# Electron-Labs/eth-lc-plonky2

Measured on AMD Instinct MI355X. Metric: lc_proofs_per_hour, higher is better.
Workload: dtype u64

## Files before the change

### eth-lc-plonky2_amd/csrc/internal.hpp

```cpp
#pragma once
#include <hip/hip_runtime.h>
#include <functional>
#include <map>
#include <string>
#include <vector>
#include "../../include/lcp2.h"
#include "gl64.hpp"
#include "ntt.hpp"

namespace lcp2 {

struct ProfFamily {
  std::vector<std::pair<hipEvent_t, hipEvent_t>> pending;
  double ms = 0;
  uint64_t launches = 0;
  double bytes = 0;
};

}

struct lcp2_ctx {
  int device = -1;
  hipStream_t stream = nullptr;
  bool own_stream = false;
  std::string last_error;
  lcp2::u64 *d_rc = nullptr;
  std::map<std::string, lcp2::u64 *> tables;
  bool prof_on = false;
  lcp2::ProfFamily fam[LCP2_K_COUNT];
  std::vector<hipEvent_t> event_pool;
  void *pin = nullptr;
  static constexpr size_t PIN_BYTES = 4u << 20;
  hipStream_t copy_stream = nullptr;
  void *scratch[4] = {nullptr, nullptr, nullptr, nullptr};
  size_t scratch_bytes[4] = {0, 0, 0, 0};

  int fail(int code, const std::string &msg) {
    last_error = msg;
    return code;
  }
};

namespace lcp2 {

#define LCP2_HIP(ctx, expr)                                                                  \
  do {                                                                                       \
    hipError_t e_ = (expr);                                                                  \
    if (e_ != hipSuccess)                                                                    \
      return (ctx)->fail(e_ == hipErrorOutOfMemory ? LCP2_E_OOM : LCP2_E_HIP,                \
                         std::string(#expr) + ": " + hipGetErrorString(e_));                 \
  } while (0)
#define LCP2_TRY(expr) do { int rc_ = (expr); if (rc_ != LCP2_OK) return rc_; } while (0)

struct DevBuf {
  void *p = nullptr;
  size_t bytes = 0;
  DevBuf() = default;
  DevBuf(const DevBuf &) = delete;
  DevBuf &operator=(const DevBuf &) = delete;
  DevBuf(DevBuf &&o) noexcept : p(o.p), bytes(o.bytes) { o.p = nullptr; o.bytes = 0; }
  DevBuf &operator=(DevBuf &&o) noexcept {
    if (this != &o) { release(); p = o.p; bytes = o.bytes; o.p = nullptr; o.bytes = 0; }
    return *this;
  }
  ~DevBuf() { release(); }
  hipError_t alloc(size_t n) {
    release();
    if (n == 0) n = 8;
    hipError_t e = hipMalloc(&p, n);
    if (e == hipSuccess) bytes = n; else p = nullptr;
    return e;
  }
  hipError_t ensure(size_t n) { return (p && bytes >= n) ? hipSuccess : alloc(n); }
  void release() { if (p) { (void)hipFree(p); p = nullptr; bytes = 0; } }
  u64 *u() const { return (u64 *)p; }
};

struct ProfScope {
  lcp2_ctx *ctx;
  int family;
  hipEvent_t a = nullptr, b = nullptr;
  ProfScope(lcp2_ctx *c, int fam, double algorithmic_bytes);
  ~ProfScope();
};

int scratch_ensure(lcp2_ctx *ctx, int slot, size_t bytes, void **out);

void launch_poseidon_permute_batch(hipStream_t s, const u64 *in, u64 *out, size_t count, const u64 *rc);
// ... 68 lines not shown
```

### eth-lc-plonky2_amd/csrc/lcp2_core.hip

```cpp
#include <cstring>
#include "internal.hpp"
#include "ntt_host.hpp"
#include "poseidon.hpp"
#include "prover_kernels.hpp"

using namespace lcp2;

extern "C" const char *lcp2_status_str(int s) {
  switch (s) {
    case LCP2_OK: return "ok";
    case LCP2_E_INVALID: return "invalid argument";
    case LCP2_E_NODEVICE: return "no usable HIP device";
    case LCP2_E_HIP: return "HIP runtime error";
    case LCP2_E_OOM: return "out of device memory";
    case LCP2_E_UNSAT: return "witness does not satisfy the circuit";
    case LCP2_E_UNSUPPORTED: return "unsupported";
    case LCP2_E_VERIFY: return "proof rejected";
    default: return "unknown status";
  }
}
extern "C" int lcp2_abi_version(void) { return LCP2_ABI_VERSION; }
extern "C" int lcp2_device_count(void) {
  int n = 0;
  if (hipGetDeviceCount(&n) != hipSuccess) return 0;
// ... 14 lines not shown
    if (d < arity_bits) return LCP2_E_INVALID;
    if (n == LCP2_MAX_FRI_LAYERS) return LCP2_E_UNSUPPORTED;
    p->fri_arity_bits[n++] = arity_bits;
    d -= arity_bits;
  }
  p->num_fri_layers = n;
  return LCP2_OK;
}
extern "C" int lcp2_params_standard(uint32_t degree_bits, uint32_t num_constants, lcp2_params *p) {
  return lcp2_params_config(degree_bits, num_constants, 3, 4, 16, 28, 4, 5, p);
}

extern "C" int lcp2_ctx_create(int device, void *stream, lcp2_ctx **out) { return lcp2_ctx_create_ex(device, stream, 0, out); }
extern "C" int lcp2_ctx_create_ex(int device, void *stream, uint32_t flags, lcp2_ctx **out) {
  if (!out) return LCP2_E_INVALID;
  *out = nullptr;
  if ((flags & ~LCP2_CTX_ORDER_WITH_DEFAULT_STREAM) || ((flags & LCP2_CTX_ORDER_WITH_DEFAULT_STREAM) && stream)) return LCP2_E_INVALID;
  int ndev = 0;
  if (hipGetDeviceCount(&ndev) != hipSuccess || ndev <= 0) return LCP2_E_NODEVICE;
  if (device < 0 || device >= ndev) return LCP2_E_INVALID;
  if (hipSetDevice(device) != hipSuccess) return LCP2_E_NODEVICE;
  lcp2_ctx *ctx = new lcp2_ctx();
  ctx->device = device;
  if (stream) {
    ctx->stream = (hipStream_t)stream;
  } else {
    const unsigned how = (flags & LCP2_CTX_ORDER_WITH_DEFAULT_STREAM) ? hipStreamDefault : hipStreamNonBlocking;
    if (hipStreamCreateWithFlags(&ctx->stream, how) != hipSuccess) { delete ctx; return LCP2_E_HIP; }
    ctx->own_stream = true;
  }
  if (hipHostMalloc(&ctx->pin, lcp2_ctx::PIN_BYTES, hipHostMallocDefault) != hipSuccess) ctx->pin = nullptr;
  u64 rc[POS_RC_WORDS];
  pos_derive_round_constants(rc);
  pos_extend_round_constants(rc);
  if (hipMalloc((void **)&ctx->d_rc, sizeof rc) != hipSuccess ||
      hipMemcpy(ctx->d_rc, rc, sizeof rc, hipMemcpyHostToDevice) != hipSuccess) {
    lcp2_ctx_destroy(ctx);
    return LCP2_E_HIP;
  }
  *out = ctx;
  return LCP2_OK;
}

extern "C" void *lcp2_ctx_stream(lcp2_ctx *ctx) { return ctx ? (void *)ctx->stream : nullptr; }

extern "C" void lcp2_ctx_destroy(lcp2_ctx *ctx) {
  if (!ctx) return;
  (void)hipSetDevice(ctx->device);
  (void)hipStreamSynchronize(ctx->stream);
  for (auto &kv : ctx->tables) (void)hipFree(kv.second);
  for (auto &f : ctx->fam)
    for (auto &pr : f.pending) { (void)hipEventDestroy(pr.first); (void)hipEventDestroy(pr.second); }
  for (auto e : ctx->event_pool) (void)hipEventDestroy(e);
  if (ctx->d_rc) (void)hipFree(ctx->d_rc);
  if (ctx->pin) (void)hipHostFree(ctx->pin);
  for (void *q : ctx->scratch) if (q) (void)hipFree(q);
  if (ctx->copy_stream) { (void)hipStreamSynchronize(ctx->copy_stream); (void)hipStreamDestroy(ctx->copy_stream); }
  if (ctx->own_stream) (void)hipStreamDestroy(ctx->stream);
  delete ctx;
}

extern "C" int lcp2_ctx_sync(lcp2_ctx *ctx) {
  if (!ctx) return LCP2_E_INVALID;
  LCP2_HIP(ctx, hipStreamSynchronize(ctx->stream));
  return LCP2_OK;
}
extern "C" const char *lcp2_last_error(lcp2_ctx *ctx) { return ctx ? ctx->last_error.c_str() : "null context"; }

namespace lcp2 {
static hipEvent_t take_event(lcp2_ctx *ctx) {
  if (!ctx->event_pool.empty()) { hipEvent_t e = ctx->event_pool.back(); ctx->event_pool.pop_back(); return e; }
  hipEvent_t e = nullptr;
  (void)hipEventCreate(&e);
  return e;
}
ProfScope::ProfScope(lcp2_ctx *c, int fam, double algorithmic_bytes) : ctx(c), family(fam) {
  if (!ctx->prof_on) return;
  a = take_event(ctx); b = take_event(ctx);
  ctx->fam[family].bytes += algorithmic_bytes;
  (void)hipEventRecord(a, ctx->stream);
}
ProfScope::~ProfScope() {
  if (!a) return;
  (void)hipEventRecord(b, ctx->stream);
  ctx->fam[family].pending.emplace_back(a, b);
}
static void prof_collect(lcp2_ctx *ctx) {
  (void)hipStreamSynchronize(ctx->stream);
  for (auto &f : ctx->fam) {
    for (auto &pr : f.pending) {
      float ms = 0;
      if (hipEventElapsedTime(&ms, pr.first, pr.second) == hipSuccess) { f.ms += ms; f.launches++; }
      ctx->event_pool.push_back(pr.first); ctx->event_pool.push_back(pr.second);
    }
    f.pending.clear();
  }
}
}

extern "C" int lcp2_prof_enable(lcp2_ctx *ctx, int on) {
  if (!ctx) return LCP2_E_INVALID;
  if (!on) prof_collect(ctx);
  ctx->prof_on = on != 0;
  return LCP2_OK;
}
extern "C" int lcp2_prof_reset(lcp2_ctx *ctx) {
// ... 434 lines not shown
```

### eth-lc-plonky2_amd/csrc/witness_rows.hip

```cpp
#include <cstring>
#include "internal.hpp"
#include "row_stage.hpp"
#include "sha_layout.hpp"
#include "sha_rows.hpp"
#include "pos_rows.hpp"
#include "prover_kernels.hpp"
#include "u32_rows.hpp"
#include "rec_rows.hpp"
#include "pos_plan.hpp"
#include "u32_plan.hpp"

using namespace lcp2;

namespace lcp2 {
int scratch_ensure(lcp2_ctx *ctx, int slot, size_t bytes, void **out) {
  if (ctx->scratch_bytes[slot] < bytes) {
    if (ctx->scratch[slot]) { LCP2_HIP(ctx, hipStreamSynchronize(ctx->stream)); LCP2_HIP(ctx, hipFree(ctx->scratch[slot])); ctx->scratch[slot] = nullptr; ctx->scratch_bytes[slot] = 0; }
    const size_t want = bytes + bytes / 4 + 4096;
    LCP2_HIP(ctx, hipMalloc(&ctx->scratch[slot], want));
    ctx->scratch_bytes[slot] = want;
  }
  *out = ctx->scratch[slot];
  return LCP2_OK;
}
}

namespace {
constexpr size_t ENDS_OK = ~(size_t)0;
size_t ends_problem(const uint32_t *ends, size_t count, size_t total) {
  if (!total) return ENDS_OK;
  for (size_t l = 0; l < count; l++)
    if (ends[l] < (l ? ends[l - 1] : 0) || ends[l] > total) return l;
  return count && ends[count - 1] == total ? ENDS_OK : count;
}
}

static_assert(sizeof(lcp2_sha_job) == sizeof(ShaJobDev) && sizeof(lcp2_cell) == sizeof(CellDev), "ABI structs must match the kernels'");

extern "C" int lcp2_sha256_witness(lcp2_ctx *ctx, const lcp2_sha_job *jobs, size_t njobs, const uint32_t *level_start, uint32_t nlevels,
                                   const uint32_t *words_in, size_t nwords, uint64_t *wires, uint64_t n, uint32_t *digests) {
  if (!ctx || !wires || (njobs && (!jobs || !level_start || nlevels == 0)) || (nwords && !words_in)) return LCP2_E_INVALID;
  if (njobs == 0) return LCP2_OK;
  if (const ShaProblem refused = sha_jobs_problem((const ShaJobDev *)jobs, njobs, level_start, nlevels, nwords, n); refused.problem)
    return ctx->fail(LCP2_E_INVALID, sha_problem_str(refused.problem));
  LCP2_HIP(ctx, hipSetDevice(ctx->device));
  void *d_jobs, *d_words, *d_rec;
  LCP2_TRY(scratch_ensure(ctx, 0, njobs * sizeof(lcp2_sha_job), &d_jobs));
  LCP2_TRY(scratch_ensure(ctx, 1, std::max<size_t>(nwords, 1) * 4, &d_words));
  LCP2_TRY(scratch_ensure(ctx, 2, njobs * (size_t)SHA_REC_WORDS * 4, &d_rec));
  Stage stage{ctx};
  LCP2_TRY(stage.behind(d_jobs, jobs, njobs * sizeof(lcp2_sha_job)));
  if (nwords) LCP2_TRY(stage.behind(d_words, words_in, nwords * 4));
  {
    ProfScope ps(ctx, LCP2_K_SHA256, 96.0 * njobs + 8.0 * 108 * SHA_ROWS * njobs);
    for (uint32_t l = 0; l < nlevels; l++)
      launch_sha_jobs_level(ctx->stream, (const ShaJobDev *)d_jobs, level_start[l], level_start[l + 1] - level_start[l],
                            (const uint32_t *)d_words, (uint32_t *)d_rec);
    launch_sha_fill_rows(ctx->stream, (const ShaJobDev *)d_jobs, (u32)njobs, (const uint32_t *)d_rec, (u64 *)wires, n);
  }
  LCP2_HIP(ctx, hipGetLastError());
  char *back = digests ? stage.room(njobs * 32) : nullptr;
  if (digests)
    LCP2_HIP(ctx, hipMemcpy2DAsync(back ? (void *)back : (void *)digests, 32, (const uint32_t *)d_rec + SHA_REC_DIGEST,
                                   (size_t)SHA_REC_WORDS * 4, 32, njobs, hipMemcpyDeviceToHost, ctx->stream));
  LCP2_HIP(ctx, hipStreamSynchronize(ctx->stream));
  if (back) memcpy(digests, back, njobs * 32);
  return LCP2_OK;
}

extern "C" int lcp2_scatter_cells(lcp2_ctx *ctx, const lcp2_cell *cells, size_t ncells, uint64_t *wires, uint64_t n) {
  if (!ctx || !wires || (ncells && !cells)) return LCP2_E_INVALID;
  if (!ncells) return LCP2_OK;
  if (scatter_cells_problem((const CellDev *)cells, ncells, n) != ncells) return ctx->fail(LCP2_E_INVALID, "scatter: row out of range");
  LCP2_HIP(ctx, hipSetDevice(ctx->device));
  void *d;
  LCP2_TRY(scratch_ensure(ctx, 3, ncells * sizeof(lcp2_cell), &d));
  LCP2_TRY(Stage{ctx}.behind(d, cells, ncells * sizeof(lcp2_cell)));
  launch_scatter_cells(ctx->stream, (const CellDev *)d, ncells, (u64 *)wires, n);
  LCP2_HIP(ctx, hipGetLastError());
  LCP2_HIP(ctx, hipStreamSynchronize(ctx->stream));
  return LCP2_OK;
}

extern "C" int lcp2_poseidon_gate_rows(lcp2_ctx *ctx, const lcp2_poseidon_row *rows, size_t nrows, uint64_t *wires, uint64_t n) {
  static_assert(sizeof(lcp2_poseidon_row) == sizeof(PoseidonRowDev), "row job layouts must agree");
  if (!ctx || !wires || (nrows && !rows)) return LCP2_E_INVALID;
  if (!nrows) return LCP2_OK;
  for (size_t i = 0; i < nrows; i++)
    if (pos_row_problem(((const PoseidonRowDev *)rows)[i], n)) return ctx->fail(LCP2_E_INVALID, "poseidon rows: row out of range or swap flag not boolean");
  LCP2_HIP(ctx, hipSetDevice(ctx->device));
  void *d;
  LCP2_TRY(scratch_ensure(ctx, 0, nrows * sizeof(lcp2_poseidon_row), &d));
  LCP2_TRY(Stage{ctx}.behind(d, rows, nrows * sizeof(lcp2_poseidon_row)));
  launch_poseidon_gate_rows(ctx->stream, (const PoseidonRowDev *)d, nrows, (u64 *)wires, n, ctx->d_rc);
  LCP2_HIP(ctx, hipGetLastError());
  LCP2_HIP(ctx, hipStreamSynchronize(ctx->stream));
  return LCP2_OK;
}

extern "C" int lcp2_u32_gate_rows(lcp2_ctx *ctx, const lcp2_u32_job *jobs, size_t njobs, lcp2_mem jobs_mem, uint64_t *wires, uint64_t n) {
  static_assert(sizeof(lcp2_u32_job) == 24 && sizeof(lcp2_u32_job) == sizeof(U32JobDev), "job layouts must agree");
  static_assert(LCP2_U32_ARITHMETIC == U32_KIND_ARITHMETIC && LCP2_U32_ADD_MANY == U32_KIND_ADD_MANY && LCP2_U32_SUBTRACTION == U32_KIND_SUBTRACTION &&
                LCP2_U32_RANGE_CHECK == U32_KIND_RANGE_CHECK && LCP2_U32_COMPARISON == U32_KIND_COMPARISON, "kind numbering must agree");
  if (!ctx || !wires || (njobs && !jobs)) return LCP2_E_INVALID;
  if (jobs_mem != LCP2_MEM_HOST && jobs_mem != LCP2_MEM_DEVICE) return ctx->fail(LCP2_E_INVALID, "u32 rows: bad lcp2_mem");
  if (!njobs) return LCP2_OK;
  const U32JobDev *list = (const U32JobDev *)jobs;
  if (jobs_mem == LCP2_MEM_HOST)
    for (size_t i = 0; i < njobs; i++)
      if (u32 problem = u32_job_problem(list[i], n))
        return ctx->fail(LCP2_E_INVALID, "u32 rows: job " + std::to_string(i) + ": " + u32_problem_str(problem));
  LCP2_HIP(ctx, hipSetDevice(ctx->device));
  RefusalFlag flag{ctx};
  LCP2_TRY(flag.begin());
  if (jobs_mem == LCP2_MEM_DEVICE) {
    launch_u32_gate_rows(ctx->stream, list, njobs, (u64 *)wires, n, flag.d);
  } else {
    constexpr size_t PIECE = (size_t)1 << 20;
    void *d;
    LCP2_TRY(scratch_ensure(ctx, 0, std::min(njobs, PIECE) * sizeof(lcp2_u32_job), &d));
    for (size_t at = 0; at < njobs; at += PIECE) {
      const size_t count = std::min(PIECE, njobs - at);
      LCP2_TRY(Stage{ctx}.behind(d, list + at, count * sizeof(lcp2_u32_job), njobs <= PIECE));
      launch_u32_gate_rows(ctx->stream, (const U32JobDev *)d, count, (u64 *)wires, n, flag.d);
    }
  }
  return flag.end("u32 rows", u32_problem_str, "the valid jobs are written");
}

namespace {
struct PlanTexts {
  const char *label, *rec_job, *written;
};

int run_plan_rows(lcp2_ctx *ctx, const lcp2_witness_plan_u32 &q, lcp2_mem lists_mem, uint64_t *wires, uint32_t ncols, uint64_t n, const PlanTexts &text) {
  const lcp2_witness_plan &p = q.base;
  const bool host = lists_mem == LCP2_MEM_HOST;
  const RecJobDev *rec = (const RecJobDev *)p.rec_jobs;
  const U32PlanJobDev *u32_jobs = (const U32PlanJobDev *)q.u32_jobs;
  const PosJobDev *pos = (const PosJobDev *)p.pos_jobs;
  const RecOperandDev *ops = (const RecOperandDev *)p.operands;
  const u32 *chain_ends = p.chain_ends;
  auto refused = [&](u32 family, u64 job, u32 problem, bool on_device) {
    return ctx->fail(LCP2_E_INVALID, std::string(text.label) + ": " + (family == 2 ? "u32 job " : family ? "poseidon job " : text.rec_job) + std::to_string(job) + ": " +
                                         (family == 2 ? u32_plan_problem_str(problem) : family ? pos_plan_problem_str(problem) : rec_problem_str(problem)) +
                                         (on_device ? std::string(" (found on the device: ") + text.written + ")" : std::string()));
  };
  if (host)
// ... 103 lines not shown
```

### eth-lc-plonky2_amd/host/builder.cpp

```cpp
#include <cstdio>
#include <algorithm>
#include <atomic>
#include <chrono>
#include <cstdlib>
#include <map>
#include <thread>
#include "host_internal.hpp"

namespace lc {

const uint32_t SHA_K[64] = {
    0x428a2f98, 0x71374491, 0xb5c0fbcf, 0xe9b5dba5, 0x3956c25b, 0x59f111f1, 0x923f82a4, 0xab1c5ed5, 0xd807aa98, 0x12835b01,
    0x243185be, 0x550c7dc3, 0x72be5d74, 0x80deb1fe, 0x9bdc06a7, 0xc19bf174, 0xe49b69c1, 0xefbe4786, 0x0fc19dc6, 0x240ca1cc,
    0x2de92c6f, 0x4a7484aa, 0x5cb0a9dc, 0x76f988da, 0x983e5152, 0xa831c66d, 0xb00327c8, 0xbf597fc7, 0xc6e00bf3, 0xd5a79147,
    0x06ca6351, 0x14292967, 0x27b70a85, 0x2e1b2138, 0x4d2c6dfc, 0x53380d13, 0x650a7354, 0x766a0abb, 0x81c2c92e, 0x92722c85,
    0xa2bfe8a1, 0xa81a664b, 0xc24b8b70, 0xc76c51a3, 0xd192e819, 0xd6990624, 0xf40e3585, 0x106aa070, 0x19a4c116, 0x1e376c08,
    0x2748774c, 0x34b0bcb5, 0x391c0cb3, 0x4ed8aa4a, 0x5b9cca4f, 0x682e6ff3, 0x748f82ee, 0x78a5636f, 0x84c87814, 0x8cc70208,
    0x90befffa, 0xa4506ceb, 0xbef9a3f7, 0xc67178f2};
const uint32_t SHA_IV[8] = {0x6a09e667, 0xbb67ae85, 0x3c6ef372, 0xa54ff53a, 0x510e527f, 0x9b05688c, 0x1f83d9ab, 0x5be0cd19};

static inline uint32_t rotr(uint32_t x, int r) { return (x >> r) | (x << (32 - r)); }

void PartialWitness::set_target(Target t, F value) { entries_.push_back({t.id, value % GOLDILOCKS_P}); }
void PartialWitness::set_hash256_target(const Hash256Target &t, const uint8_t v[32]) {
// ... 693 lines not shown
          if (backoff < 8) backoff++;
          continue;
        }
        idle.fetch_add(1, std::memory_order_acq_rel);
        while (!stop.load(std::memory_order_acquire) && epoch.load(std::memory_order_acquire) == e0) {
          if (idle.load(std::memory_order_acquire) >= active.load(std::memory_order_acquire)) stop.store(true, std::memory_order_release);
          else std::this_thread::yield();
        }
        idle.fetch_sub(1, std::memory_order_acq_rel);
      }
    } catch (...) {
      failure[k] = std::current_exception();
      stop.store(true, std::memory_order_release);
    }
    active.fetch_sub(1, std::memory_order_acq_rel);
  };
  std::vector<std::thread> threads;
  for (unsigned k = 1; k < K; k++) threads.emplace_back(lane_main, k);
  lane_main(0);
  for (auto &t : threads) t.join();
  for (unsigned k = 0; k < K; k++) if (failure[k]) std::rethrow_exception(failure[k]);
  host_ops.clear();
  for (unsigned k = 0; k < K; k++) {
    host_ops.insert(host_ops.end(), mine[k].begin(), mine[k].end());
    cells.insert(cells.end(), lane_cells[k].begin(), lane_cells[k].end());
    pos_rows.insert(pos_rows.end(), lane_rows[k].begin(), lane_rows[k].end());
  }
  std::sort(host_ops.begin(), host_ops.end());
}

void CircuitData::generate_witness_gpu(const PartialWitness &pw, std::vector<F> &public_inputs) {
  Impl *d = impl_.get();
  if (!d->gpu) throw std::runtime_error("generate_witness_gpu needs attach_gpu()");
  const uint64_t n = 1ull << desc_.params.degree_bits;
  Values V(d);
  for (auto &e : pw.entries()) V.set(e.first, e.second, "PartialWitness");
  std::vector<const Op *> host_ops, sha_ops;
  for (const Op &op : d->ops) (op.kind == Op::SHA ? sha_ops : host_ops).push_back(&op);
  std::vector<lcp2_cell> cells;
  std::vector<lcp2_poseidon_row> pos_rows;
  const bool prof = getenv("LCP2_PROF") != nullptr;
  auto now = [] { return std::chrono::steady_clock::now(); };
  auto ms = [](std::chrono::steady_clock::time_point a, std::chrono::steady_clock::time_point b) { return std::chrono::duration<double, std::milli>(b - a).count(); };
  double t_host = 0;
  if (d->host_lanes.lane_of_op.size() != d->ops.size()) {
    unsigned want = 1;
    if (const char *e = getenv("LCP2_HOST_LANES")) want = (unsigned)atoi(e);
    d->host_lanes = plan_host_lanes(d, std::max(1u, std::min(want, 8u)));
  }
  HostPhaseStats st;
  bool recording = !d->gpu_plan.ready;
  GpuWitnessPlan recorded;
  size_t n_batches = 0;
  const auto t_begin = now();
  while (true) {
    const auto t0 = now();
    run_host_phase(d, d->host_lanes, host_ops, V, cells, pos_rows, st);
    t_host += ms(t0, now());
    if (sha_ops.empty()) break;
    const size_t batch_no = n_batches++;
    if (d->gpu_plan.ready && batch_no < d->gpu_plan.batches.size()) {
      const ShaBatchPlan &B = d->gpu_plan.batches[batch_no];
      bool applies = B.ops_left.size() < sha_ops.size();
      std::vector<uint32_t> words(B.word_vars.size());
      for (size_t k = 0; k < words.size() && applies; k++) {
        if (!V.known(B.word_vars[k])) applies = false;
        else words[k] = as_u32(V.val[B.word_vars[k]], "sha256 message word");
      }
      if (applies) {
        std::vector<uint32_t> digests(B.jobs.size() * 8);
        int rc = lcp2_sha256_witness(d->ctx, B.jobs.data(), B.jobs.size(), B.level_start.data(), (uint32_t)B.level_start.size() - 1, words.data(), words.size(),
                                     (uint64_t *)d->d_wires, n, digests.data());
        if (rc != LCP2_OK) throw std::runtime_error(std::string("lcp2_sha256_witness: ") + lcp2_status_str(rc) + " (" + lcp2_last_error(d->ctx) + ")");
        for (size_t k = 0; k < B.jobs.size(); k++)
          for (int w = 0; w < 8; w++) V.set(B.out[k][w], digests[k * 8 + w], "sha256 digest");
        sha_ops.clear();
        for (uint32_t k : B.ops_left) sha_ops.push_back(&d->ops[k]);
        continue;
      }
      d->gpu_plan = GpuWitnessPlan();
      recording = false;
    }
    std::map<uint32_t, uint32_t> produced;
    std::vector<lcp2_sha_job> jobs;
    std::vector<uint32_t> level, words, word_vars;
    std::vector<const Op *> batch, later;
    for (const Op *op : sha_ops) {
      lcp2_sha_job job{};
      job.first_row = op->first_row;
      uint32_t lvl = 0;
      bool ok = true;
      size_t words_mark = words.size();
      for (int i = 0; i < 16 && ok; i++) {
        uint32_t r = d->find(op->in[i]);
        if (V.known(r)) { job.in_src[i] = (int32_t)words.size(); words.push_back(as_u32(V.val[r], "sha256 message word")); word_vars.push_back(r); }
        else {
          auto it = produced.find(r);
          if (it == produced.end()) ok = false;
          else { job.in_src[i] = ~(int32_t)it->second; lvl = std::max(lvl, level[it->second >> 3] + 1); }
        }
      }
      if (!ok) { words.resize(words_mark); word_vars.resize(words_mark); later.push_back(op); continue; }
      uint32_t slot = (uint32_t)jobs.size();
      for (int w = 0; w < 8; w++) produced[d->find(op->out8[w])] = slot * 8 + w;
      jobs.push_back(job); level.push_back(lvl); batch.push_back(op);
    }
    if (jobs.empty()) throw UnsatisfiedError("a generator is waiting for a target that is never set");
    uint32_t nlev = 0;
    for (uint32_t l : level) nlev = std::max(nlev, l + 1);
    std::vector<uint32_t> order(jobs.size()), newslot(jobs.size()), level_start(nlev + 1, 0);
    for (uint32_t l : level) level_start[l + 1]++;
    for (uint32_t l = 0; l < nlev; l++) level_start[l + 1] += level_start[l];
    {
      std::vector<uint32_t> fill(level_start.begin(), level_start.end() - 1);
      for (uint32_t s = 0; s < jobs.size(); s++) { newslot[s] = fill[level[s]]++; order[newslot[s]] = s; }
    }
    std::vector<lcp2_sha_job> sorted(jobs.size());
    for (uint32_t s = 0; s < jobs.size(); s++) {
      lcp2_sha_job j = jobs[s];
      for (int i = 0; i < 16; i++)
        if (j.in_src[i] < 0) { uint32_t ref = (uint32_t)~j.in_src[i]; j.in_src[i] = ~(int32_t)(newslot[ref >> 3] * 8 + (ref & 7)); }
      sorted[newslot[s]] = j;
    }
    std::vector<uint32_t> digests(jobs.size() * 8);
    int rc = lcp2_sha256_witness(d->ctx, sorted.data(), sorted.size(), level_start.data(), nlev, words.data(), words.size(),
                                 (uint64_t *)d->d_wires, n, digests.data());
    if (rc != LCP2_OK) throw std::runtime_error(std::string("lcp2_sha256_witness: ") + lcp2_status_str(rc) + " (" + lcp2_last_error(d->ctx) + ")");
    for (uint32_t s = 0; s < batch.size(); s++)
      for (int w = 0; w < 8; w++) V.set(batch[s]->out8[w], digests[(size_t)newslot[s] * 8 + w], "sha256 digest");
    if (recording) {
      ShaBatchPlan B;
      B.jobs = sorted; B.word_vars = word_vars; B.level_start = level_start;
      for (const Op *op : later) B.ops_left.push_back((uint32_t)(op - d->ops.data()));
      B.out.resize(jobs.size());
      for (uint32_t s = 0; s < batch.size(); s++)
        for (int w = 0; w < 8; w++) B.out[newslot[s]][w] = d->find(batch[s]->out8[w]);
      recorded.batches.push_back(std::move(B));
    }
    sha_ops.swap(later);
  }
  if (!host_ops.empty()) throw UnsatisfiedError("a generator is waiting for a target that is never set");
  const auto t_rows = now();
  int rc = lcp2_poseidon_gate_rows(d->ctx, pos_rows.data(), pos_rows.size(), (uint64_t *)d->d_wires, n);
  if (rc != LCP2_OK) throw std::runtime_error(std::string("lcp2_poseidon_gate_rows: ") + lcp2_status_str(rc) + " (" + lcp2_last_error(d->ctx) + ")");
  if (!d->gpu_plan.ready) {
    GpuWitnessPlan fresh;
    std::vector<bool> listed(d->fill_copies ? d->parent.size() : 0, false);
    for (const CellBinding &c : d->cells) {
      uint32_t g = d->gate_of_row[c.row];
      if (g == G_SHA_ADD || g == G_SHA_ROUND_A || g == G_SHA_ROUND_E || g == G_SHA_SCHED || g == G_POSEIDON) continue;
      const uint32_t root = d->find(c.var);
      if (d->fill_copies) {
        if (listed[root]) continue;
        listed[root] = true;
      }
      fresh.host_cells.push_back(CellBinding{c.row, c.col, root});
    }
    if (recording) { fresh.batches = std::move(recorded.batches); fresh.ready = true; }
    d->gpu_plan = std::move(fresh);
  }
  std::vector<lcp2_cell> &buf = d->cell_buf;
  if (buf.size() != d->gpu_plan.host_cells.size()) {
    if (d->cell_buf_pinned) { lcp2_host_unregister(d->ctx, buf.data()); d->cell_buf_pinned = false; }
    buf.resize(d->gpu_plan.host_cells.size());
    for (size_t k = 0; k < buf.size(); k++) { buf[k].row = d->gpu_plan.host_cells[k].row; buf[k].col = d->gpu_plan.host_cells[k].col; }
    if (!buf.empty()) d->cell_buf_pinned = lcp2_host_register(d->ctx, buf.data(), buf.size() * sizeof(lcp2_cell)) == LCP2_OK;
  }
  for (size_t k = 0; k < buf.size(); k++) {
    const uint32_t var = d->gpu_plan.host_cells[k].var;
    if (!V.known(var)) throw UnsatisfiedError("target has no value: wire cell");
    buf[k].value = V.val[var];
  }
  const auto t_scatter = now();
  d->cells_sent = buf.size() + cells.size();
  if (d->fill_copies) {
    rc = lcp2_witness_fill_copies(d->gpu, buf.data(), buf.size(), LCP2_MEM_HOST, (uint64_t *)d->d_wires, nullptr);
    if (rc == LCP2_OK) rc = lcp2_witness_fill_copies(d->gpu, cells.data(), cells.size(), LCP2_MEM_HOST, (uint64_t *)d->d_wires, nullptr);
    if (rc != LCP2_OK) throw std::runtime_error(std::string("lcp2_witness_fill_copies: ") + lcp2_status_str(rc) + " (" + lcp2_last_error(d->ctx) + ")");
  } else {
    rc = lcp2_scatter_cells(d->ctx, buf.data(), buf.size(), (uint64_t *)d->d_wires, n);
    if (rc == LCP2_OK) rc = lcp2_scatter_cells(d->ctx, cells.data(), cells.size(), (uint64_t *)d->d_wires, n);
    if (rc != LCP2_OK) throw std::runtime_error(std::string("lcp2_scatter_cells: ") + lcp2_status_str(rc));
  }
  if (prof)
    printf("  witness generation %.2f ms: host generators %.2f ms on %u lane(s) (%zu sweeps, %zu visits of %zu ops, %zu PoseidonGate rows), SHA-256 batches %.2f ms, "
           "PoseidonGate rows on the device + cell list %.2f ms, scatter of %zu cells %.2f ms\n",
           ms(t_begin, now()), t_host, d->host_lanes.lanes, st.sweeps, st.visits, d->ops.size(), pos_rows.size(), ms(t_begin, t_rows) - t_host, ms(t_rows, t_scatter), cells.size() + buf.size(), ms(t_scatter, now()));
  public_inputs.clear();
  for (uint32_t v : d->public_inputs) public_inputs.push_back(V.get(v, "public input"));
}

void CircuitData::set_fill_copies(bool on) {
  if (impl_->fill_copies == on) return;
  impl_->fill_copies = on;
  impl_->gpu_plan = GpuWitnessPlan();
}
size_t CircuitData::cells_sent_last() const { return impl_->cells_sent; }

void CircuitData::read_device_witness(std::vector<uint64_t> &wires) const {
  const size_t words = (size_t)desc_.params.num_wires << desc_.params.degree_bits;
  wires.resize(words);
  if (!impl_->d_wires || lcp2_buffer_read(impl_->ctx, wires.data(), impl_->d_wires, words * 8) != LCP2_OK)
    throw std::runtime_error("read_device_witness failed");
}

ProofWithPublicInputs CircuitData::prove(const PartialWitness &pw) {
  if (!impl_->gpu) throw std::runtime_error("CircuitData::prove needs attach_gpu(): there is no CPU prover in this library");
  ProofWithPublicInputs out;
  generate_witness_gpu(pw, out.public_inputs);
  out.proof.assign(lcp2_proof_words(&desc_.params), 0);
  int rc = lcp2_prove(impl_->gpu, (const uint64_t *)impl_->d_wires, LCP2_MEM_DEVICE, out.public_inputs.data(), out.public_inputs.size(),
                      out.proof.data(), out.proof.size());
  if (rc == LCP2_E_UNSAT) throw UnsatisfiedError(std::string("lcp2_prove: ") + lcp2_last_error(impl_->ctx));
  if (rc != LCP2_OK) throw std::runtime_error(std::string("lcp2_prove: ") + lcp2_status_str(rc) + " (" + lcp2_last_error(impl_->ctx) + ")");
  return out;
}

std::string CircuitData::describe_report(const lcp2_witness_report &r) const {
  if (r.gate_violations == 0 && r.copy_violations == 0) return "the witness satisfies every gate and copy constraint";
  auto cell = [](uint64_t row, uint32_t wire) { return "(" + std::to_string(row) + ", " + std::to_string(wire) + ")"; };
  std::string text;
  if (r.gate_violations) {
    const char *name = r.gate_index < desc_.gates.size() && r.gate_index < G_COUNT ? gate_name(r.gate_index) : "gate ?";
    text = "row " + std::to_string(r.gate_row) + ", gate " + name + ", constraint " + std::to_string(r.gate_constraint) + " (" +
           std::to_string(r.gate_violations) + " gate constraints violated)";
  }
  if (r.copy_violations) {
    if (!text.empty()) text += "; ";
    text += "copy constraint " + cell(r.copy_row, r.copy_wire) + " != " +
            (r.copy_to_wire == 0xFFFFFFFFu ? std::string("(no cell: the sigma value is no cell id)") : cell(r.copy_to_row, r.copy_to_wire)) + " (" +
            std::to_string(r.copy_violations) + " cells)";
  }
  return text;
}

static std::string diagnose_on_device(lcp2_ctx *ctx, lcp2_circuit *gpu, const CircuitData &data, const uint64_t *wires, lcp2_mem mem,
                                      const std::vector<F> &public_inputs) {
  lcp2_witness_report report;
  const int rc = lcp2_check_witness(gpu, wires, mem, public_inputs.data(), public_inputs.size(), &report, nullptr, 0);
// ... 57 lines not shown
```

### include/lcp2.h

```cpp
#ifndef LCP2_H
#define LCP2_H
#include <stddef.h>
#include <stdint.h>

#ifdef __cplusplus
extern "C" {
#endif

#define LCP2_ABI_VERSION 2

typedef enum {
  LCP2_OK = 0,
  LCP2_E_INVALID = -1,
  LCP2_E_NODEVICE = -2,
  LCP2_E_HIP = -3,
  LCP2_E_OOM = -4,
  LCP2_E_UNSAT = -5,
  LCP2_E_UNSUPPORTED = -6,
  LCP2_E_VERIFY = -7
} lcp2_status;

typedef enum { LCP2_MEM_HOST = 0, LCP2_MEM_DEVICE = 1 } lcp2_mem;

#define LCP2_MAX_FRI_LAYERS 8
// ... 19 lines not shown

typedef struct lcp2_ctx lcp2_ctx;
typedef struct lcp2_oracle lcp2_oracle;

const char *lcp2_status_str(int status);
int lcp2_abi_version(void);
int lcp2_device_count(void);

int lcp2_ctx_create(int device, void *stream, lcp2_ctx **out);
#define LCP2_CTX_ORDER_WITH_DEFAULT_STREAM 1u
int lcp2_ctx_create_ex(int device, void *stream, uint32_t flags, lcp2_ctx **out);
void lcp2_ctx_destroy(lcp2_ctx *ctx);
int lcp2_ctx_sync(lcp2_ctx *ctx);
void *lcp2_ctx_stream(lcp2_ctx *ctx);
const char *lcp2_last_error(lcp2_ctx *ctx);


int lcp2_poseidon_permute_batch(lcp2_ctx *ctx, const uint64_t *in, uint64_t *out, size_t count, lcp2_mem mem);

enum {
  LCP2_FIELD_MUL = 0,
  LCP2_FIELD_POW7 = 1,
  LCP2_FIELD_ADD = 2,
  LCP2_FIELD_SUB = 3,
  LCP2_FIELD_CANON = 4,
  LCP2_FIELD_ADD_LAZY = 5,
  LCP2_FIELD_SUB_LAZY = 6,
  LCP2_FIELD_SHL = 16
};
int lcp2_field_op_batch(lcp2_ctx *ctx, const uint64_t *a, const uint64_t *b, uint64_t *out, size_t count, uint32_t op, lcp2_mem mem);

int lcp2_merkle_cap(lcp2_ctx *ctx, const uint64_t *leaves, size_t nleaves, size_t leaf_len,
                    uint32_t cap_height, lcp2_mem mem, uint64_t *cap );

int lcp2_ntt_batch(lcp2_ctx *ctx, uint64_t *data, size_t ncols, uint32_t log_n, int inverse,
                   uint64_t shift, lcp2_mem mem);

int lcp2_lde_batch(lcp2_ctx *ctx, const uint64_t *coeffs, uint64_t *out, size_t ncols, uint32_t log_n,
                   uint32_t rate_bits, lcp2_mem mem);

int lcp2_sha256_tree(lcp2_ctx *ctx, const uint8_t *leaves, uint32_t height, size_t trees,
                     uint8_t *nodes, uint32_t *round_trace, lcp2_mem mem);

typedef struct {
  uint32_t first_row;
  int32_t in_src[16];
} lcp2_sha_job;
typedef struct {
  uint32_t row, col;
  uint64_t value;
} lcp2_cell;
int lcp2_sha256_witness(lcp2_ctx *ctx, const lcp2_sha_job *jobs, size_t njobs, const uint32_t *level_start, uint32_t nlevels,
                        const uint32_t *words_in, size_t nwords, uint64_t *wires, uint64_t n, uint32_t *digests);
int lcp2_scatter_cells(lcp2_ctx *ctx, const lcp2_cell *cells, size_t ncells, uint64_t *wires, uint64_t n);
typedef struct {
  uint32_t row;
  uint32_t swap;
  uint64_t in[12];
} lcp2_poseidon_row;
int lcp2_poseidon_gate_rows(lcp2_ctx *ctx, const lcp2_poseidon_row *rows, size_t nrows, uint64_t *wires, uint64_t n);
enum { LCP2_U32_ARITHMETIC = 0, LCP2_U32_ADD_MANY = 1, LCP2_U32_SUBTRACTION = 2, LCP2_U32_RANGE_CHECK = 3, LCP2_U32_COMPARISON = 4 };
typedef struct {
  uint32_t row;
  uint16_t kind;
  uint16_t op;
  uint32_t in[4];
} lcp2_u32_job;
int lcp2_u32_gate_rows(lcp2_ctx *ctx, const lcp2_u32_job *jobs, size_t njobs, lcp2_mem jobs_mem,
                       uint64_t *wires , uint64_t n);

enum { LCP2_REC_ARITHMETIC = 0, LCP2_REC_BASE_SUM, LCP2_REC_ARITHMETIC_EXT, LCP2_REC_MUL_EXT, LCP2_REC_REDUCING,
       LCP2_REC_REDUCING_EXT, LCP2_REC_POSEIDON_MDS, LCP2_REC_RANDOM_ACCESS, LCP2_REC_EXPONENTIATION,
       LCP2_REC_COSET_INTERPOLATION, LCP2_REC_KINDS };
enum { LCP2_REC_IMM = 0, LCP2_REC_CELL = 1 };
typedef struct {
  uint64_t v;
  uint32_t col;
  uint32_t src;
} lcp2_rec_operand;
typedef struct {
  uint32_t row;
  uint16_t kind;
  uint16_t op;
  uint32_t first_operand, reserved;
} lcp2_rec_job;
int lcp2_rec_gate_rows(lcp2_ctx *ctx, const lcp2_rec_job *jobs, size_t njobs,
                       const lcp2_rec_operand *operands, size_t noperands,
                       const uint32_t *level_ends , size_t nlevels,
                       lcp2_mem lists_mem ,
                       uint64_t *wires , uint32_t ncols, uint64_t n);

enum { LCP2_PLAN_IMM = 0, LCP2_PLAN_CELL = 1, LCP2_PLAN_PREV = 2 };
typedef struct { uint32_t row, first_operand; } lcp2_pos_job;
typedef struct {
  const lcp2_rec_job *rec_jobs;  size_t nrec;    const uint32_t *rec_level_ends;
  const lcp2_pos_job *pos_jobs;  size_t npos;
  const uint32_t *chain_ends;    size_t nchains;
  const uint32_t *pos_level_ends;
  const lcp2_rec_operand *operands; size_t noperands;
  size_t nlevels;
} lcp2_witness_plan;
int lcp2_witness_plan_rows(lcp2_ctx *ctx, const lcp2_witness_plan *plan, lcp2_mem lists_mem,
                           uint64_t *wires , uint32_t ncols, uint64_t n);

typedef struct { uint32_t row; uint16_t kind , op; uint32_t first_operand, reserved; } lcp2_u32_plan_job;
typedef struct {
  lcp2_witness_plan base;
  const lcp2_u32_plan_job *u32_jobs; size_t nu32;
  const uint32_t *u32_level_ends;
} lcp2_witness_plan_u32;
int lcp2_witness_plan_rows_u32(lcp2_ctx *ctx, const lcp2_witness_plan_u32 *plan, lcp2_mem lists_mem,
                               uint64_t *wires , uint32_t ncols, uint64_t n);

// ... 204 lines not shown
```

Before: 9350.

## Overlap host cell-value gathering with SHA-256 witness batches and merge syncs

The SHA-256 witness call is split into begin/end, so the host fills the known wire-cell values into the pinned cell buffer while the device runs the SHA batch. Cells whose values are not yet known are tracked in a late list and retried on later passes. The PoseidonGate rows and the host-cell scatter are now queued together behind one stream synchronize instead of two. This adds per-context pending state and more complex bookkeeping on the host in exchange for less serial host work and fewer syncs.

```diff
diff --git a/eth-lc-plonky2_amd/csrc/internal.hpp b/eth-lc-plonky2_amd/csrc/internal.hpp
--- a/eth-lc-plonky2_amd/csrc/internal.hpp
+++ b/eth-lc-plonky2_amd/csrc/internal.hpp
@@ -34,6 +34,13 @@
   hipStream_t copy_stream = nullptr;
   void *scratch[4] = {nullptr, nullptr, nullptr, nullptr};
   size_t scratch_bytes[4] = {0, 0, 0, 0};
+  hipEvent_t sha_done = nullptr;
+  struct ShaPending {
+    bool open = false;
+    const char *staged = nullptr;
+    uint32_t *digests = nullptr;
+    size_t bytes = 0;
+  } sha_pending;
 
   int fail(int code, const std::string &msg) {
     last_error = msg;
diff --git a/eth-lc-plonky2_amd/csrc/lcp2_core.hip b/eth-lc-plonky2_amd/csrc/lcp2_core.hip
--- a/eth-lc-plonky2_amd/csrc/lcp2_core.hip
+++ b/eth-lc-plonky2_amd/csrc/lcp2_core.hip
@@ -90,6 +90,7 @@
   for (auto &f : ctx->fam)
     for (auto &pr : f.pending) { (void)hipEventDestroy(pr.first); (void)hipEventDestroy(pr.second); }
   for (auto e : ctx->event_pool) (void)hipEventDestroy(e);
+  if (ctx->sha_done) (void)hipEventDestroy(ctx->sha_done);
   if (ctx->d_rc) (void)hipFree(ctx->d_rc);
   if (ctx->pin) (void)hipHostFree(ctx->pin);
   for (void *q : ctx->scratch) if (q) (void)hipFree(q);
diff --git a/eth-lc-plonky2_amd/csrc/witness_rows.hip b/eth-lc-plonky2_amd/csrc/witness_rows.hip
--- a/eth-lc-plonky2_amd/csrc/witness_rows.hip
+++ b/eth-lc-plonky2_amd/csrc/witness_rows.hip
@@ -37,9 +37,10 @@
 
 static_assert(sizeof(lcp2_sha_job) == sizeof(ShaJobDev) && sizeof(lcp2_cell) == sizeof(CellDev), "ABI structs must match the kernels'");
 
-extern "C" int lcp2_sha256_witness(lcp2_ctx *ctx, const lcp2_sha_job *jobs, size_t njobs, const uint32_t *level_start, uint32_t nlevels,
-                                   const uint32_t *words_in, size_t nwords, uint64_t *wires, uint64_t n, uint32_t *digests) {
+extern "C" int lcp2_sha256_witness_begin(lcp2_ctx *ctx, const lcp2_sha_job *jobs, size_t njobs, const uint32_t *level_start, uint32_t nlevels,
+                                         const uint32_t *words_in, size_t nwords, uint64_t *wires, uint64_t n, uint32_t *digests) {
   if (!ctx || !wires || (njobs && (!jobs || !level_start || nlevels == 0)) || (nwords && !words_in)) return LCP2_E_INVALID;
+  if (ctx->sha_pending.open) return ctx->fail(LCP2_E_INVALID, "sha256 witness: the batch begun before has not been ended");
   if (njobs == 0) return LCP2_OK;
   if (const ShaProblem refused = sha_jobs_problem((const ShaJobDev *)jobs, njobs, level_start, nlevels, nwords, n); refused.problem)
     return ctx->fail(LCP2_E_INVALID, sha_problem_str(refused.problem));
@@ -51,6 +52,8 @@
   Stage stage{ctx};
   LCP2_TRY(stage.behind(d_jobs, jobs, njobs * sizeof(lcp2_sha_job)));
   if (nwords) LCP2_TRY(stage.behind(d_words, words_in, nwords * 4));
+  if (!ctx->sha_done) LCP2_HIP(ctx, hipEventCreateWithFlags(&ctx->sha_done, hipEventDisableTiming));
+  char *back = digests ? stage.room(njobs * 32) : nullptr;
   {
     ProfScope ps(ctx, LCP2_K_SHA256, 96.0 * njobs + 8.0 * 108 * SHA_ROWS * njobs);
     for (uint32_t l = 0; l < nlevels; l++)
@@ -59,41 +62,92 @@
     launch_sha_fill_rows(ctx->stream, (const ShaJobDev *)d_jobs, (u32)njobs, (const uint32_t *)d_rec, (u64 *)wires, n);
   }
   LCP2_HIP(ctx, hipGetLastError());
-  char *back = digests ? stage.room(njobs * 32) : nullptr;
   if (digests)
     LCP2_HIP(ctx, hipMemcpy2DAsync(back ? (void *)back : (void *)digests, 32, (const uint32_t *)d_rec + SHA_REC_DIGEST,
                                    (size_t)SHA_REC_WORDS * 4, 32, njobs, hipMemcpyDeviceToHost, ctx->stream));
-  LCP2_HIP(ctx, hipStreamSynchronize(ctx->stream));
-  if (back) memcpy(digests, back, njobs * 32);
-  return LCP2_OK;
+  LCP2_HIP(ctx, hipEventRecord(ctx->sha_done, ctx->stream));
+  ctx->sha_pending = {true, back, digests, njobs * 32};
+  return LCP2_OK;
+}
+
+extern "C" int lcp2_sha256_witness_end(lcp2_ctx *ctx) {
+  if (!ctx) return LCP2_E_INVALID;
+  if (!ctx->sha_pending.open) return LCP2_OK;
+  const lcp2_ctx::ShaPending p = ctx->sha_pending;
+  ctx->sha_pending = {};
+  LCP2_HIP(ctx, hipSetDevice(ctx->device));
+  LCP2_HIP(ctx, hipEventSynchronize(ctx->sha_done));
+  if (p.staged) memcpy(p.digests, p.staged, p.bytes);
+  return LCP2_OK;
+}
+
+extern "C" int lcp2_sha256_witness(lcp2_ctx *ctx, const lcp2_sha_job *jobs, size_t njobs, const uint32_t *level_start, uint32_t nlevels,
+                                   const uint32_t *words_in, size_t nwords, uint64_t *wires, uint64_t n, uint32_t *digests) {
+  LCP2_TRY(lcp2_sha256_witness_begin(ctx, jobs, njobs, level_start, nlevels, words_in, nwords, wires, n, digests));
+  return lcp2_sha256_witness_end(ctx);
+}
+
+namespace {
+int cells_refused(lcp2_ctx *ctx, const lcp2_cell *cells, size_t ncells, uint64_t n) {
+  if (scatter_cells_problem((const CellDev *)cells, ncells, n) != ncells) return ctx->fail(LCP2_E_INVALID, "scatter: row out of range");
+  return LCP2_OK;
+}
+int queue_cells(lcp2_ctx *ctx, Stage &stage, const lcp2_cell *cells, size_t ncells, uint64_t *wires, uint64_t n) {
+  void *d;
+  LCP2_TRY(scratch_ensure(ctx, 3, ncells * sizeof(lcp2_cell), &d));
+  LCP2_TRY(stage.behind(d, cells, ncells * sizeof(lcp2_cell)));
+  launch_scatter_cells(ctx->stream, (const CellDev *)d, ncells, (u64 *)wires, n);
+  LCP2_HIP(ctx, hipGetLastError());
+  return LCP2_OK;
+}
+int poseidon_rows_refused(lcp2_ctx *ctx, const lcp2_poseidon_row *rows, size_t nrows, uint64_t n) {
+  static_assert(sizeof(lcp2_poseidon_row) == sizeof(PoseidonRowDev), "row job layouts must agree");
+  for (size_t i = 0; i < nrows; i++)
+    if (pos_row_problem(((const PoseidonRowDev *)rows)[i], n)) return ctx->fail(LCP2_E_INVALID, "poseidon rows: row out of range or swap flag not boolean");
+  return LCP2_OK;
+}
+int queue_poseidon_rows(lcp2_ctx *ctx, Stage &stage, const lcp2_poseidon_row *rows, size_t nrows, uint64_t *wires, uint64_t n) {
+  void *d;
+  LCP2_TRY(scratch_ensure(ctx, 0, nrows * sizeof(lcp2_poseidon_row), &d));
+  LCP2_TRY(stage.behind(d, rows, nrows * sizeof(lcp2_poseidon_row)));
+  launch_poseidon_gate_rows(ctx->stream, (const PoseidonRowDev *)d, nrows, (u64 *)wires, n, ctx->d_rc);
+  LCP2_HIP(ctx, hipGetLastError());
+  return LCP2_OK;
+}
 }
 
 extern "C" int lcp2_scatter_cells(lcp2_ctx *ctx, const lcp2_cell *cells, size_t ncells, uint64_t *wires, uint64_t n) {
   if (!ctx || !wires || (ncells && !cells)) return LCP2_E_INVALID;
   if (!ncells) return LCP2_OK;
-  if (scatter_cells_problem((const CellDev *)cells, ncells, n) != ncells) return ctx->fail(LCP2_E_INVALID, "scatter: row out of range");
-  LCP2_HIP(ctx, hipSetDevice(ctx->device));
-  void *d;
-  LCP2_TRY(scratch_ensure(ctx, 3, ncells * sizeof(lcp2_cell), &d));
-  LCP2_TRY(Stage{ctx}.behind(d, cells, ncells * sizeof(lcp2_cell)));
-  launch_scatter_cells(ctx->stream, (const CellDev *)d, ncells, (u64 *)wires, n);
-  LCP2_HIP(ctx, hipGetLastError());
+  LCP2_TRY(cells_refused(ctx, cells, ncells, n));
+  LCP2_HIP(ctx, hipSetDevice(ctx->device));
+  Stage stage{ctx};
+  LCP2_TRY(queue_cells(ctx, stage, cells, ncells, wires, n));
   LCP2_HIP(ctx, hipStreamSynchronize(ctx->stream));
   return LCP2_OK;
 }
 
 extern "C" int lcp2_poseidon_gate_rows(lcp2_ctx *ctx, const lcp2_poseidon_row *rows, size_t nrows, uint64_t *wires, uint64_t n) {
-  static_assert(sizeof(lcp2_poseidon_row) == sizeof(PoseidonRowDev), "row job layouts must agree");
   if (!ctx || !wires || (nrows && !rows)) return LCP2_E_INVALID;
   if (!nrows) return LCP2_OK;
-  for (size_t i = 0; i < nrows; i++)
-    if (pos_row_problem(((const PoseidonRowDev *)rows)[i], n)) return ctx->fail(LCP2_E_INVALID, "poseidon rows: row out of range or swap flag not boolean");
-  LCP2_HIP(ctx, hipSetDevice(ctx->device));
-  void *d;
-  LCP2_TRY(scratch_ensure(ctx, 0, nrows * sizeof(lcp2_poseidon_row), &d));
-  LCP2_TRY(Stage{ctx}.behind(d, rows, nrows * sizeof(lcp2_poseidon_row)));
-  launch_poseidon_gate_rows(ctx->stream, (const PoseidonRowDev *)d, nrows, (u64 *)wires, n, ctx->d_rc);
-  LCP2_HIP(ctx, hipGetLastError());
+  LCP2_TRY(poseidon_rows_refused(ctx, rows, nrows, n));
+  LCP2_HIP(ctx, hipSetDevice(ctx->device));
+  Stage stage{ctx};
+  LCP2_TRY(queue_poseidon_rows(ctx, stage, rows, nrows, wires, n));
+  LCP2_HIP(ctx, hipStreamSynchronize(ctx->stream));
+  return LCP2_OK;
+}
+
+extern "C" int lcp2_poseidon_rows_and_cells(lcp2_ctx *ctx, const lcp2_poseidon_row *rows, size_t nrows, const lcp2_cell *cells, size_t ncells,
+                                            uint64_t *wires, uint64_t n) {
+  if (!ctx || !wires || (nrows && !rows) || (ncells && !cells)) return LCP2_E_INVALID;
+  if (!nrows && !ncells) return LCP2_OK;
+  LCP2_TRY(poseidon_rows_refused(ctx, rows, nrows, n));
+  LCP2_TRY(cells_refused(ctx, cells, ncells, n));
+  LCP2_HIP(ctx, hipSetDevice(ctx->device));
+  Stage stage{ctx};
+  if (nrows) LCP2_TRY(queue_poseidon_rows(ctx, stage, rows, nrows, wires, n));
+  if (ncells) LCP2_TRY(queue_cells(ctx, stage, cells, ncells, wires, n));
   LCP2_HIP(ctx, hipStreamSynchronize(ctx->stream));
   return LCP2_OK;
 }
diff --git a/eth-lc-plonky2_amd/host/builder.cpp b/eth-lc-plonky2_amd/host/builder.cpp
--- a/eth-lc-plonky2_amd/host/builder.cpp
+++ b/eth-lc-plonky2_amd/host/builder.cpp
@@ -769,6 +769,27 @@
   bool recording = !d->gpu_plan.ready;
   GpuWitnessPlan recorded;
   size_t n_batches = 0;
+  std::vector<lcp2_cell> &buf = d->cell_buf;
+  std::vector<uint32_t> late;
+  bool cells_swept = false;
+  auto restart_cells = [&] { cells_swept = false; late.clear(); };
+  auto refresh_known_cells = [&] {
+    const std::vector<CellBinding> &planned = d->gpu_plan.host_cells;
+    auto fill = [&](uint32_t k) {
+      const uint32_t var = planned[k].var;
+      if (!V.known(var)) return false;
+      buf[k].value = V.val[var];
+      return true;
+    };
+    if (!cells_swept) {
+      for (uint32_t k = 0; k < planned.size(); k++) if (!fill(k)) late.push_back(k);
+      cells_swept = true;
+    } else {
+      size_t kept = 0;
+      for (uint32_t k : late) if (!fill(k)) late[kept++] = k;
+      late.resize(kept);
+    }
+  };
   const auto t_begin = now();
   while (true) {
     const auto t0 = now();
@@ -786,8 +807,12 @@
       }
       if (applies) {
         std::vector<uint32_t> digests(B.jobs.size() * 8);
-        int rc = lcp2_sha256_witness(d->ctx, B.jobs.data(), B.jobs.size(), B.level_start.data(), (uint32_t)B.level_start.size() - 1, words.data(), words.size(),
-                                     (uint64_t *)d->d_wires, n, digests.data());
+        int rc = lcp2_sha256_witness_begin(d->ctx, B.jobs.data(), B.jobs.size(), B.level_start.data(), (uint32_t)B.level_start.size() - 1, words.data(),
+                                           words.size(), (uint64_t *)d->d_wires, n, digests.data());
+        if (rc == LCP2_OK) {
+          if (buf.size() == d->gpu_plan.host_cells.size()) refresh_known_cells();
+          rc = lcp2_sha256_witness_end(d->ctx);
+        }
         if (rc != LCP2_OK) throw std::runtime_error(std::string("lcp2_sha256_witness: ") + lcp2_status_str(rc) + " (" + lcp2_last_error(d->ctx) + ")");
         for (size_t k = 0; k < B.jobs.size(); k++)
           for (int w = 0; w < 8; w++) V.set(B.out[k][w], digests[k * 8 + w], "sha256 digest");
@@ -797,6 +822,7 @@
       }
       d->gpu_plan = GpuWitnessPlan();
       recording = false;
+      restart_cells();
     }
     std::map<uint32_t, uint32_t> produced;
     std::vector<lcp2_sha_job> jobs;
@@ -858,9 +884,8 @@
   }
   if (!host_ops.empty()) throw UnsatisfiedError("a generator is waiting for a target that is never set");
   const auto t_rows = now();
-  int rc = lcp2_poseidon_gate_rows(d->ctx, pos_rows.data(), pos_rows.size(), (uint64_t *)d->d_wires, n);
-  if (rc != LCP2_OK) throw std::runtime_error(std::string("lcp2_poseidon_gate_rows: ") + lcp2_status_str(rc) + " (" + lcp2_last_error(d->ctx) + ")");
   if (!d->gpu_plan.ready) {
+    restart_cells();
     GpuWitnessPlan fresh;
     std::vector<bool> listed(d->fill_copies ? d->parent.size() : 0, false);
     for (const CellBinding &c : d->cells) {
@@ -876,32 +901,32 @@
     if (recording) { fresh.batches = std::move(recorded.batches); fresh.ready = true; }
     d->gpu_plan = std::move(fresh);
   }
-  std::vector<lcp2_cell> &buf = d->cell_buf;
   if (buf.size() != d->gpu_plan.host_cells.size()) {
+    restart_cells();
     if (d->cell_buf_pinned) { lcp2_host_unregister(d->ctx, buf.data()); d->cell_buf_pinned = false; }
     buf.resize(d->gpu_plan.host_cells.size());
     for (size_t k = 0; k < buf.size(); k++) { buf[k].row = d->gpu_plan.host_cells[k].row; buf[k].col = d->gpu_plan.host_cells[k].col; }
     if (!buf.empty()) d->cell_buf_pinned = lcp2_host_register(d->ctx, buf.data(), buf.size() * sizeof(lcp2_cell)) == LCP2_OK;
   }
-  for (size_t k = 0; k < buf.size(); k++) {
-    const uint32_t var = d->gpu_plan.host_cells[k].var;
-    if (!V.known(var)) throw UnsatisfiedError("target has no value: wire cell");
-    buf[k].value = V.val[var];
-  }
+  refresh_known_cells();
+  if (!late.empty()) throw UnsatisfiedError("target has no value: wire cell");
   const auto t_scatter = now();
   d->cells_sent = buf.size() + cells.size();
+  int rc;
   if (d->fill_copies) {
+    rc = lcp2_poseidon_gate_rows(d->ctx, pos_rows.data(), pos_rows.size(), (uint64_t *)d->d_wires, n);
+    if (rc != LCP2_OK) throw std::runtime_error(std::string("lcp2_poseidon_gate_rows: ") + lcp2_status_str(rc) + " (" + lcp2_last_error(d->ctx) + ")");
     rc = lcp2_witness_fill_copies(d->gpu, buf.data(), buf.size(), LCP2_MEM_HOST, (uint64_t *)d->d_wires, nullptr);
     if (rc == LCP2_OK) rc = lcp2_witness_fill_copies(d->gpu, cells.data(), cells.size(), LCP2_MEM_HOST, (uint64_t *)d->d_wires, nullptr);
     if (rc != LCP2_OK) throw std::runtime_error(std::string("lcp2_witness_fill_copies: ") + lcp2_status_str(rc) + " (" + lcp2_last_error(d->ctx) + ")");
   } else {
-    rc = lcp2_scatter_cells(d->ctx, buf.data(), buf.size(), (uint64_t *)d->d_wires, n);
+    rc = lcp2_poseidon_rows_and_cells(d->ctx, pos_rows.data(), pos_rows.size(), buf.data(), buf.size(), (uint64_t *)d->d_wires, n);
     if (rc == LCP2_OK) rc = lcp2_scatter_cells(d->ctx, cells.data(), cells.size(), (uint64_t *)d->d_wires, n);
-    if (rc != LCP2_OK) throw std::runtime_error(std::string("lcp2_scatter_cells: ") + lcp2_status_str(rc));
+    if (rc != LCP2_OK) throw std::runtime_error(std::string("lcp2_poseidon_rows_and_cells / lcp2_scatter_cells: ") + lcp2_status_str(rc) + " (" + lcp2_last_error(d->ctx) + ")");
   }
   if (prof)
     printf("  witness generation %.2f ms: host generators %.2f ms on %u lane(s) (%zu sweeps, %zu visits of %zu ops, %zu PoseidonGate rows), SHA-256 batches %.2f ms, "
-           "PoseidonGate rows on the device + cell list %.2f ms, scatter of %zu cells %.2f ms\n",
+           "cell list behind the digests %.2f ms, PoseidonGate rows on the device + scatter of %zu cells %.2f ms\n",
            ms(t_begin, now()), t_host, d->host_lanes.lanes, st.sweeps, st.visits, d->ops.size(), pos_rows.size(), ms(t_begin, t_rows) - t_host, ms(t_rows, t_scatter), cells.size() + buf.size(), ms(t_scatter, now()));
   public_inputs.clear();
   for (uint32_t v : d->public_inputs) public_inputs.push_back(V.get(v, "public input"));
diff --git a/include/lcp2.h b/include/lcp2.h
--- a/include/lcp2.h
+++ b/include/lcp2.h
@@ -95,6 +95,9 @@
 } lcp2_cell;
 int lcp2_sha256_witness(lcp2_ctx *ctx, const lcp2_sha_job *jobs, size_t njobs, const uint32_t *level_start, uint32_t nlevels,
                         const uint32_t *words_in, size_t nwords, uint64_t *wires, uint64_t n, uint32_t *digests);
+int lcp2_sha256_witness_begin(lcp2_ctx *ctx, const lcp2_sha_job *jobs, size_t njobs, const uint32_t *level_start, uint32_t nlevels,
+                              const uint32_t *words_in, size_t nwords, uint64_t *wires, uint64_t n, uint32_t *digests);
+int lcp2_sha256_witness_end(lcp2_ctx *ctx);
 int lcp2_scatter_cells(lcp2_ctx *ctx, const lcp2_cell *cells, size_t ncells, uint64_t *wires, uint64_t n);
 typedef struct {
   uint32_t row;
@@ -102,6 +105,8 @@
   uint64_t in[12];
 } lcp2_poseidon_row;
 int lcp2_poseidon_gate_rows(lcp2_ctx *ctx, const lcp2_poseidon_row *rows, size_t nrows, uint64_t *wires, uint64_t n);
+int lcp2_poseidon_rows_and_cells(lcp2_ctx *ctx, const lcp2_poseidon_row *rows, size_t nrows, const lcp2_cell *cells, size_t ncells,
+                                 uint64_t *wires, uint64_t n);
 enum { LCP2_U32_ARITHMETIC = 0, LCP2_U32_ADD_MANY = 1, LCP2_U32_SUBTRACTION = 2, LCP2_U32_RANGE_CHECK = 3, LCP2_U32_COMPARISON = 4 };
 typedef struct {
   uint32_t row;
```

After: 9322. About the same (-0.3%).
